# WangYuTum/odometry

Measured on AMD Instinct MI355X. Metric: tracked frames/sec (1241x376, 4-level pyramid), higher is better.
Workload: dtype f32

## Files before the change

### __graft_entry__.py

```python
import os
import sys

ROOT = os.path.dirname(os.path.abspath(__file__))
if ROOT not in sys.path:
    sys.path.insert(0, ROOT)


def build():
    import subprocess
    from odometry_amd import build as b
    b.build(force=False, verbose=True)
    from oracle import oracle
    oracle.build()
    subprocess.check_call(["g++", "-O2", "-std=c++17", "-ffp-contract=off", "-fno-fast-math", "-mfma", "-shared", "-fPIC",
                           "-o", os.path.join(ROOT, "tests", "_build_hostemu.so"), os.path.join(ROOT, "tests", "hostemu.cpp")])
    import importlib.util
    spec = importlib.util.spec_from_file_location("devmath", os.path.join(ROOT, "tests", "devmath.py"))
    devmath = importlib.util.module_from_spec(spec)
    spec.loader.exec_module(devmath)
    devmath.build_all(verbose=True)
    import odometry_amd
    from odometry_amd import _lib
    _lib.load()


def smoke():
    import numpy as np
    from odometry_amd import api, synth
    from oracle import oracle as O
    seq = synth.make_sequence(2, seed=5, with_depth=True)
    L0, L1, R1 = seq["left"][0], seq["left"][1], seq["right"][1]
    inv = synth.semi_dense_inverse_depth(seq["depth"][0], L0)
    p0, d0, p1 = api.ImagePyramid(4, L0, True), api.DepthPyramid(4, inv, False), api.ImagePyramid(4, L1, True)
    for l, ref in enumerate(O.image_pyramid(L1, 4, True)):
        assert np.array_equal(p1.GetPyramidImage(l), ref), f"pyramid level {l} differs from the oracle"
    lm = api.LevenbergMarquardtOptimizer(0.01, 0.995, [10, 20, 30, 30], np.eye(4), None, 1, 28.0)
    T = lm.Solve(p0, d0, p1)
    ref = O.lm_solve(O.image_pyramid(L0, flat=True), O.depth_pyramid(inv, flat=True), O.image_pyramid(L1, flat=True),
                     376, 1241, O.lm_params())
    assert lm.last_status == 0 and ref["status"] == 0
    err = float(np.abs(T.astype(np.float64) - ref["pose"]).max())
    assert err < 1e-5, f"pose differs from the oracle by {err}"
    de = api.DepthEstimator(8.0, 900.0, 15.0, 0.1, 30.0, 0.01, 28.0, 0.995, 50, 4, None, None,
                            float(np.float32(386.1448) / np.float32(718.856)), 80000)
    val = np.zeros(L1.shape, np.uint8)
    disp = np.zeros(L1.shape, np.float32)
    dep = np.zeros(L1.shape, np.float32)
    st = de.ComputeDepth(L1, R1, val, disp, dep)
    rd = O.compute_depth(L1, R1, O.depth_params())
    assert st == rd["status"] == 0
    assert np.array_equal(disp, rd["disp"]) and np.array_equal(val, rd["val"])
    print(f"smoke ok: pose max|d|={err:.2e}, evals={lm.launch_stats()[0]}, valid depth={int(val.sum())}")


if __name__ == "__main__":
    build()
    if len(sys.argv) > 1 and sys.argv[1] == "smoke":
        smoke()
```

### odometry_amd/csrc/kernels.hip.h

```cpp
#pragma once
#include <hip/hip_runtime.h>
#include "odo_math.h"

#ifndef ODO_PHASE_STAMPS
#define ODO_PHASE_STAMPS 0
#endif
#if ODO_PHASE_STAMPS
#define ODO_DBG(a) ((a).dbg)
#else
#define ODO_DBG(a) ((unsigned long long*)nullptr)
#endif

#ifndef ODO_KERNEL
#define ODO_KERNEL __global__
#define ODO_KERNEL_T __global__
#endif
#ifdef ODO_LM_CHAIN_TU
#define ODO_DEVICE_VAR static __device__
#else
#define ODO_DEVICE_VAR __device__
#endif

namespace odo {

// ... 987 lines not shown
    if (pending) need_step = lm_decide(&s, acc_sh, precision);
    if (smdbg) { c1 = __builtin_readcyclecounter(); c2 = c1; c3 = c1; }
    if (need_step) {
      float d[6];
      solve_damped_wave_regs(acc_sh, s.lambda, d);
#pragma unroll
      for (int i = 0; i < 6; i++) s.delta[i] = d[i];
      if (smdbg) { asm volatile("" ::"v"(d[0]), "v"(d[5])); c2 = __builtin_readcyclecounter(); }
#ifdef ODO_NO_LANE_SINCOS
      lm_apply_step(&s, s.max_iters);
#else
      lm_apply_step_wave(&s, s.max_iters);
#endif
      if (smdbg) { asm volatile("" ::"v"(s.T[0]), "v"(s.T[14])); c3 = __builtin_readcyclecounter(); }
    }
    if (smdbg && t == 0) { smdbg[0] += c1 - c0; smdbg[1] += c2 - c1; smdbg[2] += c3 - c2; smdbg[3] += 1; }
    if (pending) {
      if (publisher && t == 0 && trace) {
        const int ev = s.n_evals - 1;
        if (ev < kTraceCap) {
          LmTraceRow& r = trace[ev];
          r.level = lvl0;
          r.iter = iter0;
          r.n_res = (int)acc_sh[28];
          r.err = s.err_now;
          r.accepted = (s.status == 0 && !(s.err_now > err_last0)) ? 1 : 0;
          r.stop = (s.stop_reason == 3 || s.active) ? 0 : s.stop_reason;
          r.lambda_after = s.lambda;
#pragma unroll
          for (int i = 0; i < 6; i++) r.delta[i] = (s.active || s.stop_reason == 3) ? s.delta[i] : 0.0f;
        }
        int evals_this_level = 0;
#pragma unroll
        for (int i = 0; i < 8; i++) evals_this_level += (i == (lvl0 & 7)) ? s.iters_level[i] : 0;
        if (iter0 == 0 && evals_this_level == 1) cost_stat[lvl0 * 2 + 0] = s.err_now;
        cost_stat[lvl0 * 2 + 1] = s.err_now;
      }
      s.pending = 0;
    }
    if (lv) {
      while (!s.active && s.status == 0 && !s.finished) {
        const int next = (s.level < 0) ? n_levels - 1 : s.level - 1;
        if (next < stop_level) { s.finished = 1; break; }
        s.stop_reason = 0;
        lm_begin_level(&s, next, lambda0, lv[next].max_iters);
      }
      if (s.status != 0) s.finished = 1;
    }
    if (t == 0) s_sh = s;
  }
  __syncthreads();
}

struct LmHot {
  Se3 cur, inc;
  float Tc[12];
  float lambda, err_last;
  int level, iter, max_iters, active, status, finished, n_evals, stop_reason;
};
__device__ __forceinline__ void lm_hot_load(LmHot& h, const LmState& s) {
  h.cur = s.cur; h.inc = s.inc;
  float M[16];
  se3_to_colmajor(s.cur, M);
#pragma unroll
  for (int c = 0; c < 4; c++)
#pragma unroll
    for (int r = 0; r < 3; r++) h.Tc[c * 3 + r] = M[c * 4 + r];
  h.lambda = s.lambda; h.err_last = s.err_last;
  h.level = s.level; h.iter = s.iter; h.max_iters = s.max_iters; h.active = s.active; h.status = s.status; h.finished = s.finished;
  h.n_evals = s.n_evals; h.stop_reason = s.stop_reason;
}
__device__ __forceinline__ void lm_hot_store(const LmHot& h, LmState& s) {
  s.cur = h.cur; s.inc = h.inc; s.last = h.cur;
  s.lambda = h.lambda; s.err_last = h.err_last;
  s.level = h.level; s.iter = h.iter; s.max_iters = h.max_iters; s.active = h.active; s.status = h.status; s.finished = h.finished;
  s.n_evals = h.n_evals; s.stop_reason = h.stop_reason;
  s.pending = 0;
}
__device__ __forceinline__ void lm_state_machine_hot(LmHot& h, const StepLevel* lv, int n_levels, float lambda0, float precision,
                                                     LmState& s_sh, const double* acc_sh, LmTraceRow* __restrict__ trace,
                                                     float* __restrict__ cost_stat, bool publisher,
                                                     unsigned long long* smdbg = nullptr, int stop_level = 0) {
  const int t = threadIdx.x;
  if (t < 64) {
    unsigned long long c0 = smdbg ? __builtin_readcyclecounter() : 0, c1 = c0, c2 = c0, c3 = c0;
    const int iter0 = h.iter, lvl0 = h.level;
    const float err_last0 = h.err_last;
    float Tprev[12];
#pragma unroll
    for (int c = 0; c < 4; c++)
#pragma unroll
      for (int r = 0; r < 3; r++) Tprev[c * 3 + r] = s_sh.T[c * 4 + r];
    h.n_evals++;
    if (t == 0) s_sh.iters_level[lvl0 & 7] += 1;
    bool need_step = false;
    float err_now = 0.0f;
    bool have_err = false;
    if (!(acc_sh[28] > 0.0)) {
      h.status = -1;
      h.active = 0;
    } else {
      err_now = (float)(acc_sh[27] / acc_sh[28]);
      have_err = true;
      if (err_now > h.err_last) {
        h.lambda = h.lambda * 5.0f;
        if (h.lambda > 1e+5f) { h.active = 0; h.stop_reason = 2; }
        else need_step = true;
      } else {
        h.cur = h.inc;
#pragma unroll
        for (int i = 0; i < 12; i++) h.Tc[i] = Tprev[i];
        const float err_diff = err_now / h.err_last;
        if (err_diff > precision) { h.active = 0; h.stop_reason = 1; }
        else {
          h.err_last = err_now;
          h.lambda = fmaxf(h.lambda / 5.0f, 1e-5f);
          need_step = true;
        }
      }
    }
    if (smdbg) { c1 = __builtin_readcyclecounter(); c2 = c1; c3 = c1; }
    float d[6] = {0.0f, 0.0f, 0.0f, 0.0f, 0.0f, 0.0f};
    bool new_T = false;
    float Tn[16];
#pragma unroll
    for (int i = 0; i < 16; i++) Tn[i] = 0.0f;
    if (need_step) {
      solve_damped_wave_regs(acc_sh, h.lambda, d);
      if (smdbg) { asm volatile("" ::"v"(d[0]), "v"(d[5])); c2 = __builtin_readcyclecounter(); }
      Se3 dd;
      se3_exp_wave(d, &dd);
      const float C[16] = {h.Tc[0], h.Tc[1], h.Tc[2], 0.0f, h.Tc[3], h.Tc[4], h.Tc[5], 0.0f,
                           h.Tc[6], h.Tc[7], h.Tc[8], 0.0f, h.Tc[9], h.Tc[10], h.Tc[11], 1.0f};
      se3_left_update_mat(dd, C, &h.inc);
      se3_to_colmajor(h.inc, Tn);
      new_T = true;
      h.iter++;
      if (!(h.max_iters > h.iter)) { h.active = 0; h.stop_reason = 3; }
      if (smdbg) { asm volatile("" ::"v"(Tn[0]), "v"(Tn[14])); c3 = __builtin_readcyclecounter(); }
    }
    if (smdbg && t == 0) { smdbg[0] += c1 - c0; smdbg[1] += c2 - c1; smdbg[2] += c3 - c2; smdbg[3] += 1; }
    if (t == 0) {
      if (have_err) s_sh.err_now = err_now;
      if (need_step) {
#pragma unroll
        for (int i = 0; i < 6; i++) s_sh.delta[i] = d[i];
      }
    }
    if (publisher && t == 0 && trace) {
      const int ev = h.n_evals - 1;
      const float e = s_sh.err_now;
      if (ev < kTraceCap) {
        LmTraceRow& r = trace[ev];
        r.level = lvl0;
        r.iter = iter0;
        r.n_res = (int)acc_sh[28];
        r.err = e;
        r.accepted = (h.status == 0 && !(e > err_last0)) ? 1 : 0;
        r.stop = (h.stop_reason == 3 || h.active) ? 0 : h.stop_reason;
        r.lambda_after = h.lambda;
#pragma unroll
        for (int i = 0; i < 6; i++) r.delta[i] = (h.active || h.stop_reason == 3) ? d[i] : 0.0f;
      }
      const int evals_this_level = s_sh.iters_level[lvl0 & 7];
      if (iter0 == 0 && evals_this_level == 1) cost_stat[lvl0 * 2 + 0] = e;
      cost_stat[lvl0 * 2 + 1] = e;
    }
    if (lv) {
      while (!h.active && h.status == 0 && !h.finished) {
        const int next = (h.level < 0) ? n_levels - 1 : h.level - 1;
        if (next < stop_level) { h.finished = 1; break; }
        h.stop_reason = 0;
        h.level = next;
        h.iter = 0;
        h.err_last = 1e+10f;
        h.lambda = lambda0;
        h.inc = h.cur;
        h.max_iters = lv[next].max_iters;
        h.active = (h.status == 0 && h.max_iters > 0) ? 1 : 0;
#pragma unroll
        for (int c = 0; c < 4; c++) {
#pragma unroll
          for (int r = 0; r < 3; r++) Tn[c * 4 + r] = h.Tc[c * 3 + r];
          Tn[c * 4 + 3] = (c == 3) ? 1.0f : 0.0f;
        }
        new_T = true;
      }
      if (h.status != 0) h.finished = 1;
    }
    if (t == 0) {
      if (new_T) {
#pragma unroll
        for (int i = 0; i < 16; i++) s_sh.T[i] = Tn[i];
      }
      s_sh.level = h.level; s_sh.active = h.active; s_sh.status = h.status; s_sh.finished = h.finished;
    }
  }
  __syncthreads();
}

constexpr int kUpdThreads = 1024;
#define ODO_STAMP(i) do { if (STAMP && threadIdx.x == 0) stamps[i] = __builtin_readcyclecounter(); } while (0)
template <bool STAMP>
__device__ __forceinline__ void lm_update_body(LmState* __restrict__ st, const double* __restrict__ partials,
                                               int nblk, int expect_level, float precision, int max_iters,
                                               LmTraceRow* __restrict__ trace, float* __restrict__ cost_stat,
                                               int* __restrict__ host_prog, int seq,
                                               unsigned long long* __restrict__ stamps) {
  ODO_STAMP(0);
  if (!(st->active != 0 && st->level == expect_level)) {
    if (host_prog && threadIdx.x == 0) __hip_atomic_store(host_prog, seq, __ATOMIC_RELAXED, __HIP_MEMORY_SCOPE_SYSTEM);
    return;
  }
  __shared__ double sh[32][32];
  __shared__ double acc_sh[32];
  __shared__ LmState s_sh;
  const int t = threadIdx.x;
  const int q = t & 31, seg = t >> 5;
  double v = 0.0;
  if (q < ODO_NACC) {
    double v0 = 0.0, v1 = 0.0, v2 = 0.0, v3 = 0.0;
    int b = seg;
    for (; b + 96 < nblk; b += 128) {
      v0 += partials[(size_t)b * ODO_NACC + q];
      v1 += partials[(size_t)(b + 32) * ODO_NACC + q];
      v2 += partials[(size_t)(b + 64) * ODO_NACC + q];
      v3 += partials[(size_t)(b + 96) * ODO_NACC + q];
    }
    for (; b < nblk; b += 32) v0 += partials[(size_t)b * ODO_NACC + q];
    v = (v0 + v1) + (v2 + v3);
  }
  ODO_STAMP(1);
  sh[seg][q] = v;
  if (t < (int)(sizeof(LmState) / sizeof(int))) ((int*)&s_sh)[t] = ((const int*)st)[t];
  __syncthreads();
  if (t < ODO_NACC) {
    double a = 0.0;
#pragma unroll
    for (int g = 0; g < 32; g++) a += sh[g][t];
    acc_sh[t] = a;
  }
  if (t == 0) s_sh.max_iters = max_iters;
  __syncthreads();
  ODO_STAMP(2);
  lm_state_machine(true, nullptr, 0, 0.0f, precision, s_sh, acc_sh, trace, cost_stat, true);
  ODO_STAMP(3); ODO_STAMP(4); ODO_STAMP(5); ODO_STAMP(6);
  if (t < (int)(sizeof(LmState) / sizeof(int))) ((int*)st)[t] = ((const int*)&s_sh)[t];
  if (t == 0) {
    const LmState& s = s_sh;
    if (host_prog) {
      if (!s.active) __hip_atomic_store(host_prog + 2 + expect_level, 1, __ATOMIC_RELAXED, __HIP_MEMORY_SCOPE_SYSTEM);
// ... 254 lines not shown
  lm_span_begin(q.span);
  __shared__ LmState s_sh;
  extern __shared__ __attribute__((aligned(16))) double red_sh[];
  __shared__ double acc_sh[32];
  __shared__ StepLevel lv_sh[ODO_MAX_LEVELS_K];
  __shared__ unsigned long long sm_sh[4];
  unsigned long long arm_g0 = 0;
  if (kArmed && threadIdx.x < 17) arm_g0 = __hip_atomic_load(a.arm + threadIdx.x, __ATOMIC_RELAXED, __HIP_MEMORY_SCOPE_SYSTEM);
  lm_copy_levels(lv_sh, lv_src);
  if (threadIdx.x == 0) {
#pragma unroll
    for (int i = 0; i < 4; i++) sm_sh[i] = 0;
  }
  __shared__ __attribute__((aligned(16))) float arm_pose_sh[16];
  __shared__ __attribute__((aligned(16))) int arm_verdict_sh4[4];
  if (kArmed) {
    if (threadIdx.x < 64) {
      const int lane = (int)threadIdx.x;
      unsigned long long g = arm_g0;
      bool got = __all(lane >= 17 || (int)(g >> 32) == a.token);
      const unsigned long long t0 = (unsigned long long)wall_clock64();
      for (int spin = 0; !got; spin++) {
        if (lane < 17) g = __hip_atomic_load(a.arm + lane, __ATOMIC_RELAXED, __HIP_MEMORY_SCOPE_SYSTEM);
        got = __all(lane >= 17 || (int)(g >> 32) == a.token);
        if (!got && (spin & 15) == 15 && (unsigned long long)wall_clock64() - t0 > (a.fine_wait ? (unsigned long long)a.fine_wait : kArmWaitTicks)) break;
      }
      if (lane < 16) arm_pose_sh[lane] = __uint_as_float((unsigned)g);
      if (lane == 16) arm_verdict_sh4[0] = got ? (int)(unsigned)g : 3;
    }
    __syncthreads();
    if (arm_verdict_sh4[0] == 3) {
      if (threadIdx.x < 64) {
        if (threadIdx.x < (int)(sizeof(LmState) / sizeof(int))) ((int*)&s_sh)[threadIdx.x] = 0;
        if (threadIdx.x == 0) { s_sh.status = -2; s_sh.active = 0; s_sh.finished = 1; }
      }
      __syncthreads();
      lm_fused_publish(s_sh, q.st_out, a.host_prog, q.seq, a.token, a.cost_stat, a.out, a.done_flag, a.final_state);
      return;
    }
    if (arm_verdict_sh4[0] != 1) return;
  } else {
    __syncthreads();
  }
#if ODO_PHASE_STAMPS
  const unsigned long long w_p1 = (unsigned long long)wall_clock64();
#endif
  lm_fused_prologue(q.st_in, q.part_in, lv_sh, a.n_levels, a.lambda0, a.precision, s_sh, red_sh, acc_sh, (kFull ? a.trace : (LmTraceRow*)nullptr), a.cost_stat, true,
                    kArmed ? arm_pose_sh : (q.first_of_solve ? a.init : nullptr), a.stop_level, (!kArmed && a.chain_in_token) ? a.chain_pose : nullptr);
#if ODO_PHASE_STAMPS
  const unsigned long long w_p2 = (unsigned long long)wall_clock64();
#endif
  LmHot hot;
  lm_hot_load(hot, s_sh);
  if (ODO_DBG(a) && threadIdx.x == 0 && q.seq < 56) ODO_DBG(a)[16 + 2 * q.seq] = wall_clock64();
  unsigned long long c_eval = 0, c_red = 0, c_sm = 0, c_it = 0, c_last = ODO_DBG(a) ? __builtin_readcyclecounter() : 0;
  const unsigned long long c_begin = c_last, w_begin = ODO_DBG(a) ? (unsigned long long)wall_clock64() : 0;
  auto lap = [&](unsigned long long& sum) {
    if (ODO_DBG(a)) { const unsigned long long now = __builtin_readcyclecounter(); sum += now - c_last; c_last = now; }
  };
  static_assert(kCoarseBlock == 2 * kLmBlock, "two 256-point virtual blocks per round");
  constexpr int kS = 8;
  constexpr int kVbMax = (kCoarseMaxPoints + kLmBlock - 1) / kLmBlock;
  __shared__ double part_sh[kVbMax][32];
  __shared__ double sc_part[2][kCoarseChunks];
  __shared__ int sc_cnt[kCoarseChunks];
  const int tl = threadIdx.x & (kLmBlock - 1), half = threadIdx.x >> 8;
  float* rows_sh = (float*)red_sh + half * (kRowFloats * RowBuf<kLmBlock>::W);
  const int my_q = tl / kS, my_s = tl % kS;
  int rowA = 0, rowB = 0;
  if (my_q < ODO_NACC) rows_of_quantity(my_q, &rowA, &rowB);
  PointK cpt[kCoarseRounds];
  bool cpt_ok[kCoarseRounds] = {false, false};
  int cpt_level = -1;
  for (int guard = 0; guard < 4096; guard++) {
    const bool run = (s_sh.active != 0 && s_sh.status == 0 && s_sh.level >= min_level);
    if (!run) break;
    c_it++;
    const StepLevel& L = lv_sh[s_sh.level];
    const float* I2u = lm_uniform_ptr(L.I2);
    float T[16];
#pragma unroll
    for (int i = 0; i < 16; i++) T[i] = s_sh.T[i];
    const int nvb = L.nblk;
    if (s_sh.level != cpt_level) {
      cpt_level = s_sh.level;
#pragma unroll
      for (int rd = 0; rd < kCoarseRounds; rd++) {
        const int vb = 2 * rd + half, idx = vb * kLmBlock + tl;
        cpt_ok[rd] = vb < nvb && idx < L.n;
        if (cpt_ok[rd]) cpt[rd] = load_point(L.pl, idx);
      }
    }
    float td_r[kCoarseRounds] = {0.0f, 0.0f}, td_J[kCoarseRounds][6] = {{0.0f, 0.0f, 0.0f, 0.0f, 0.0f, 0.0f}, {0.0f, 0.0f, 0.0f, 0.0f, 0.0f, 0.0f}};
    bool td_valid[kCoarseRounds] = {false, false};
    float td_scale_sqr = 1.0f;
    if ((kFull && a.robust == 2)) {
      float e2[kCoarseRounds];
#pragma unroll
      for (int rd = 0; rd < kCoarseRounds; rd++) {
        if (cpt_ok[rd]) td_valid[rd] = point_residual_g<kFull>(cpt[rd], T, L.k, I2u, L.rows, L.cols, &td_r[rd], td_J[rd]);
        e2[rd] = td_r[rd] * td_r[rd];
      }
      const float sg = coarse_tdist_sigma(sc_part, sc_cnt, e2, td_valid, (nvb + 1) / 2);
      td_scale_sqr = sg * sg;
    }
#pragma unroll
    for (int vb0 = 0; vb0 < 2 * kCoarseRounds; vb0 += 2) {
      if (vb0 >= nvb) break;
      const int vb = vb0 + half;
      float r = 0.0f, w = 0.0f, J[6] = {0.0f, 0.0f, 0.0f, 0.0f, 0.0f, 0.0f};
      bool valid = false;
      if ((kFull && a.robust == 2)) {
        r = td_r[vb0 / 2]; valid = td_valid[vb0 / 2];
#pragma unroll
        for (int i = 0; i < 6; i++) J[i] = td_J[vb0 / 2][i];
        if (valid) w = robust_weight(r, 2, a.huber_delta, td_scale_sqr);
      } else if (cpt_ok[vb0 / 2]) {
        if (point_residual_g<kFull>(cpt[vb0 / 2], T, L.k, I2u, L.rows, L.cols, &r, J)) {
          w = robust_weight(r, kFull ? a.robust : (a.robust == 1 ? 1 : 0), a.huber_delta, 1.0f);
          valid = true;
        }
      }
      if (vb0 > 0) __syncthreads();
      rows_store_z(rows_sh, RowBuf<kLmBlock>::W, tl, J, w, r, valid);
      __syncthreads();
      if (vb0 == 0) lap(c_eval);
      double accq = 0.0;
      if (vb < nvb) {
        if (my_q < ODO_NACC) accq = rows_accumulate<kLmBlock, kS>(rows_sh, rowA, rowB, my_s, accq);
        accq = rows_butterfly8(accq);
      }
      if (nvb == 1) {
        if (half == 0 && my_q < ODO_NACC && my_s == 0) {
          double v = 0.0;
          v += accq;
          double acc = 0.0;
          acc += v;
#pragma unroll
          for (int g = 1; g < 8; g++) acc += 0.0;
          acc_sh[my_q] = acc;
        }
      } else if (vb < nvb && my_q < ODO_NACC && my_s == 0) {
        part_sh[vb][my_q] = accq;
      }
    }
    __syncthreads();
    if (nvb > 1) {
      const int fq = threadIdx.x & 31, fseg = threadIdx.x >> 5;
      double* fold_sh = red_sh;
      if (fseg < 8) {
        double v = 0.0;
        if (fq < ODO_NACC)
          for (int b = fseg; b < nvb; b += 8) v += part_sh[b][fq];
        fold_sh[fseg * 32 + fq] = v;
      }
      __syncthreads();
      if (threadIdx.x < ODO_NACC) {
        double acc = 0.0;
#pragma unroll
        for (int g = 0; g < 8; g++) acc += fold_sh[g * 32 + threadIdx.x];
        acc_sh[threadIdx.x] = acc;
      }
    }
    lap(c_red);
    lm_state_machine_hot(hot, lv_sh, a.n_levels, a.lambda0, a.precision, s_sh, acc_sh, (kFull ? a.trace : (LmTraceRow*)nullptr), a.cost_stat, true,
                         ODO_DBG(a) ? sm_sh : nullptr, a.stop_level);
    lap(c_sm);
  }
#if ODO_PHASE_STAMPS
  const unsigned long long w_loop_end = (unsigned long long)wall_clock64();
#endif
  if (threadIdx.x == 0) lm_hot_store(hot, s_sh);
  lm_fused_publish(s_sh, q.st_out, a.host_prog, q.seq, a.token, a.cost_stat, a.out, a.done_flag, a.final_state, chain_out_of(a));
#if ODO_PHASE_STAMPS
  if (ODO_DBG(a) && threadIdx.x == 0) {
    const unsigned long long now = (unsigned long long)wall_clock64();
    g_lm_diag[4] += w_begin - w_entry; g_lm_diag[5] += w_loop_end - w_begin; g_lm_diag[6] += now - w_loop_end;
    g_lm_diag[16] += w_p1 - w_entry; g_lm_diag[17] += w_p2 - w_p1; g_lm_diag[18] += w_begin - w_p2;
    if (g_lm_diag[1] && w_entry > g_lm_diag[1] && w_entry - g_lm_diag[1] < 100000ull) { g_lm_diag[7] += w_entry - g_lm_diag[1]; g_lm_diag[3] += w_entry - g_lm_diag[2]; g_lm_diag[14] += 1; }
    g_lm_diag[0] = now; g_lm_diag[8] += 1;
  }
#endif
  if (ODO_DBG(a) && threadIdx.x == 0) {
    if (q.seq < 56) ODO_DBG(a)[16 + 2 * q.seq + 1] = wall_clock64();
    ODO_DBG(a)[0] += c_eval; ODO_DBG(a)[1] += c_red; ODO_DBG(a)[2] += c_sm; ODO_DBG(a)[3] += c_it;
    ODO_DBG(a)[4] += __builtin_readcyclecounter() - c_begin; ODO_DBG(a)[5] += 1;
    ODO_DBG(a)[6] += (unsigned long long)wall_clock64() - w_begin;
#pragma unroll
    for (int i = 0; i < 4; i++) ODO_DBG(a)[8 + i] += sm_sh[i];
  }
  lm_span_end(q.span);
}

#ifdef ODO_LM_CHAIN_TU
static __global__ void __launch_bounds__(kCoarseBlock) lm_coarse_kernel(StepArgs a, int min_level) {
  const StepLaunch q = {a.st_in, a.st_out, a.part_in, a.part_out, a.seq, a.first_of_solve, a.span};
  lm_coarse_body<false>(a, q, min_level, lm_kernarg_words());
}
static __global__ void __launch_bounds__(kCoarseBlock) lm_coarse_armed_kernel(StepArgs a, int min_level) {
  const StepLaunch q = {a.st_in, a.st_out, a.part_in, a.part_out, a.seq, a.first_of_solve, a.span};
  lm_coarse_body<false, true>(a, q, min_level, lm_kernarg_words());
}
static __global__ void __launch_bounds__(kCoarseBlock) lm_coarse_full_kernel(StepArgs a, int min_level) {
  const StepLaunch q = {a.st_in, a.st_out, a.part_in, a.part_out, a.seq, a.first_of_solve, a.span};
  lm_coarse_body<true>(a, q, min_level, lm_kernarg_words());
}
#endif
template <bool kFull>
__device__ __forceinline__ void lm_coarse_batch_entry(const StepArgs* __restrict__ table, int seq, int first_of_solve, unsigned long long* span) {
  const StepArgs& a = table[blockIdx.y];
  const StepLaunch q = {a.st2[seq & 1], a.st2[(seq + 1) & 1], a.part2[seq & 1], a.part2[(seq + 1) & 1], seq, first_of_solve, span};
  lm_coarse_body<kFull>(a, q, a.min_level, (const unsigned*)&table[blockIdx.y]);
}
ODO_KERNEL void __launch_bounds__(kCoarseBlock) lm_coarse_kernel_batch(const StepArgs* __restrict__ table, int seq, int first_of_solve,
                                                                       unsigned long long* span) {
  lm_coarse_batch_entry<false>(table, seq, first_of_solve, span);
}
ODO_KERNEL void __launch_bounds__(kCoarseBlock) lm_coarse_full_kernel_batch(const StepArgs* __restrict__ table, int seq, int first_of_solve,
                                                                            unsigned long long* span) {
  lm_coarse_batch_entry<true>(table, seq, first_of_solve, span);
}

constexpr int kFineGran = 2 * ODO_NACC;
constexpr int kFineRowsMax = 160;
constexpr int kFineChunk = 8;
// ... 197 lines not shown
  return sigma;
}
template <bool kTdist, bool kTrace>
__device__ __forceinline__ void lm_fine_body(const StepArgs& a, const StepLaunch& q, int K, int w, unsigned long long* __restrict__ xbuf,
                                             int fault, int lo_level, const unsigned* __restrict__ lv_src) {
#if ODO_PHASE_STAMPS
  const unsigned long long w_entry = (unsigned long long)wall_clock64();
#endif
  __builtin_amdgcn_s_setprio(3);
  const int t = threadIdx.x, tl = t & (kLmBlock - 1), half = t >> 8;
  const bool publisher = (w == 0);
  if (publisher && t == 0 && q.span) atomicMin(q.span, (unsigned long long)wall_clock64());
  __shared__ LmState s_sh;
  __shared__ double fold_sh[8 * 32];
  __shared__ double acc_sh[32];
  __shared__ StepLevel lv_sh[ODO_MAX_LEVELS_K];
  __shared__ float rows_sh2[2][kRowFloats * RowBuf<kLmBlock>::W];
  __shared__ int bail_sh, local_sh;
  __shared__ unsigned long long sm_sh[4];
  float* rows_sh = rows_sh2[half];
  const unsigned tag_base = a.fine_epoch << 8;
  unsigned long long* place = xbuf + 2 * kFineRowsMax * kFineGran;
  const unsigned wait_limit = a.fine_wait ? a.fine_wait : kFineWaitTicks;
  lm_copy_levels(lv_sh, lv_src);
  if (t == 0) {
    bail_sh = 0;
    local_sh = 0;
#pragma unroll
    for (int i = 0; i < 4; i++) sm_sh[i] = 0;
    __hip_atomic_store(place + w, ((unsigned long long)(unsigned)fine_xcc_id() << 32) | tag_base, __ATOMIC_RELAXED, __HIP_MEMORY_SCOPE_AGENT);
  }
  __syncthreads();
  lm_fused_prologue(q.st_in, q.part_in, lv_sh, a.n_levels, a.lambda0, a.precision, s_sh, fold_sh, acc_sh, (kTrace ? a.trace : (LmTraceRow*)nullptr), a.cost_stat,
                    publisher, q.first_of_solve ? a.init : nullptr, a.stop_level, a.chain_in_token ? a.chain_pose : nullptr);
  LmHot hot;
  lm_hot_load(hot, s_sh);
  if (t < 64) {
    bool same = true, got = false;
    if (t < K) {
      unsigned long long pw = 0;
      const FineDeadline dl = FineDeadline::begin(wait_limit);
      for (int spin = 0; !got; spin++) {
        pw = __hip_atomic_load(place + t, __ATOMIC_RELAXED, __HIP_MEMORY_SCOPE_AGENT);
        got = ((unsigned)pw == tag_base);
        if (!got && dl.expired(spin)) break;
      }
      same = got && ((int)(pw >> 32) == fine_xcc_id());
    } else {
      got = true;
    }
    const bool all_got = __all(got), all_same = __all(same);
    if (t == 0) { local_sh = (all_got && all_same) ? 1 : 0; if (!all_got) bail_sh = 1; }
  }
  __syncthreads();
  const bool local = local_sh != 0;
  constexpr int kS = 8;
  const int my_q = tl / kS, my_s = tl % kS;
  int rowA = 0, rowB = 0;
  if (my_q < ODO_NACC) rows_of_quantity(my_q, &rowA, &rowB);
  const int fq = t & 31, fseg = t >> 5;
  PointK pt;
  bool pt_ok = false;
  int pt_level = -1;
  unsigned long long c_eval = 0, c_xchg = 0, c_sm = 0, c_it = 0, c_last = ODO_DBG(a) ? __builtin_readcyclecounter() : 0;
#if ODO_PHASE_STAMPS
  unsigned long long c_first = 0, n_first = 0;
#endif
  const unsigned long long c_begin = c_last, w_begin = ODO_DBG(a) ? (unsigned long long)wall_clock64() : 0;
  auto lap = [&](unsigned long long& sum) {
    if (ODO_DBG(a)) { const unsigned long long now = __builtin_readcyclecounter(); sum += now - c_last; c_last = now; }
  };
  for (int ev = 0; ev < 4096; ev++) {
    const bool run = (s_sh.active != 0 && s_sh.status == 0 && !s_sh.finished && !bail_sh && s_sh.level >= lo_level);
    if (!run) break;
    c_it++;
    const StepLevel& L = lv_sh[s_sh.level];
    const float* I2u = lm_uniform_ptr(L.I2);
    const int nblk = L.nblk;
    const unsigned tag = tag_base + 1u + (unsigned)(ev % 255);
    unsigned long long* buf = xbuf + (size_t)(ev & 1) * kFineRowsMax * kFineGran;
    float T[16];
#pragma unroll
    for (int i = 0; i < 16; i++) T[i] = s_sh.T[i];
#if ODO_PHASE_STAMPS
    const bool first_of_level = (s_sh.level != pt_level);
#endif
    const bool resident = (nblk <= 2 * K) && (L.n <= nblk * kLmBlock);
    if (resident) {
      const int vb = w + half * K;
      if (s_sh.level != pt_level) {
        pt_level = s_sh.level;
        const int idx = vb * kLmBlock + tl;
        pt_ok = vb < nblk && idx < L.n;
        if (pt_ok) pt = load_point(L.pl, idx);
      }
      float r = 0.0f, wgt = 0.0f, J[6] = {0.0f, 0.0f, 0.0f, 0.0f, 0.0f, 0.0f};
      bool valid = false;
      if (pt_ok && point_residual_g<kTdist || kTrace>(pt, T, L.k, I2u, L.rows, L.cols, &r, J)) {
        wgt = robust_weight(r, (kTdist || kTrace) ? a.robust : (a.robust == 1 ? 1 : 0), a.huber_delta, 1.0f);
        valid = true;
      }
      if (kTdist && w < nblk) {
        __shared__ double td_ws_sh[2][8];
        __shared__ int td_cnt_sh[8];
        const float sg = fine_tdist_sigma(xbuf + kFineScaleOff, vb * 4 + (tl >> 6), 4 * nblk,
                                          ((a.fine_epoch & 0xfffu) << 20) | (((unsigned)ev & 0x3ffu) << 10), r * r, valid, local, wait_limit, &bail_sh,
                                          td_ws_sh, td_cnt_sh);
        if (valid) wgt = robust_weight(r, 2, a.huber_delta, sg * sg);
      }
      rows_store_z(rows_sh, RowBuf<kLmBlock>::W, tl, J, wgt, r, valid);
      __syncthreads();
      if (bail_sh) break;
      if (vb < nblk) {
        double accq = 0.0;
        if (my_q < ODO_NACC) accq = rows_accumulate<kLmBlock, kS>(rows_sh, rowA, rowB, my_s, accq);
        accq = rows_butterfly8(accq);
        if (my_q < ODO_NACC && my_s == 0 && !(fault && vb == 0)) fine_publish(buf, vb, my_q, accq, tag, local);
      }
    } else {
      const int rounds = (L.n + nblk * kLmBlock - 1) / (nblk * kLmBlock);
      for (int vb0 = w; vb0 < nblk; vb0 += 2 * K) {
        const int vb = vb0 + half * K;
        double accq = 0.0;
        for (int rd = 0; rd < rounds; rd++) {
          const int idx = (vb + rd * nblk) * kLmBlock + tl;
          float r = 0.0f, wgt = 0.0f, J[6] = {0.0f, 0.0f, 0.0f, 0.0f, 0.0f, 0.0f};
          bool valid = false;
          if (vb < nblk && idx < L.n) {
            const PointK p = load_point(L.pl, idx);
            if (point_residual_g<kTdist || kTrace>(p, T, L.k, I2u, L.rows, L.cols, &r, J)) {
              wgt = robust_weight(r, (kTdist || kTrace) ? a.robust : (a.robust == 1 ? 1 : 0), a.huber_delta, 1.0f);
              valid = true;
            }
          }
          __syncthreads();
          rows_store_z(rows_sh, RowBuf<kLmBlock>::W, tl, J, wgt, r, valid);
          __syncthreads();
          if (my_q < ODO_NACC) accq = rows_accumulate<kLmBlock, kS>(rows_sh, rowA, rowB, my_s, accq);
        }
        accq = rows_butterfly8(accq);
        if (vb < nblk && my_q < ODO_NACC && my_s == 0 && !(fault && vb == 0)) fine_publish(buf, vb, my_q, accq, tag, local);
      }
    }
#if ODO_PHASE_STAMPS
    { const unsigned long long before = c_eval; lap(c_eval); if (first_of_level) { c_first += c_eval - before; n_first++; } }
#else
    lap(c_eval);
#endif
    double v = 0.0;
    __builtin_amdgcn_s_setprio(0);
    if (fq < ODO_NACC && fseg < 8) {
      for (int b0 = fseg; b0 < nblk; b0 += 8 * kFineChunk) {
        FineG2 g2[kFineChunk];
        bool all = false;
        FineDeadline dl = {0ull, 0ull, wait_limit};
        for (int spin = 0; !all; spin++) {
          if (spin == 1) dl = FineDeadline::begin(wait_limit);
          if (spin > 0) { if (dl.expired(spin)) break; __builtin_amdgcn_s_sleep(1); }
          all = true;
#pragma unroll
          for (int u = 0; u < kFineChunk; u++) {
            const int b = b0 + 8 * u;
            if (b < nblk) g2[u] = *(const volatile FineG2Global*)(buf + (size_t)b * kFineGran + 2 * fq);
          }
#pragma unroll
          for (int u = 0; u < kFineChunk; u++) {
            const int b = b0 + 8 * u;
            if (b < nblk) all = all && (g2[u].x == tag) && (g2[u].z == tag);
          }
        }
        if (!all) bail_sh = 1;
#pragma unroll
        for (int u = 0; u < kFineChunk; u++) {
          const int b = b0 + 8 * u;
          if (b < nblk) v += __longlong_as_double((long long)(((unsigned long long)g2[u].y << 32) | (unsigned long long)g2[u].w));
        }
      }
    }
    __builtin_amdgcn_s_setprio(3);
    if (fseg < 8) fold_sh[fseg * 32 + fq] = v;
    __syncthreads();
    if (t < ODO_NACC) {
      double acc = 0.0;
#pragma unroll
      for (int g = 0; g < 8; g++) acc += fold_sh[g * 32 + t];
      acc_sh[t] = acc;
    }
    lap(c_xchg);
    if (bail_sh) break;
    lm_state_machine_hot(hot, lv_sh, a.n_levels, a.lambda0, a.precision, s_sh, acc_sh, (kTrace ? a.trace : (LmTraceRow*)nullptr), a.cost_stat, publisher,
                         (ODO_DBG(a) && publisher) ? sm_sh : nullptr, a.stop_level);
    lap(c_sm);
  }
#if ODO_PHASE_STAMPS
  const unsigned long long w_loop_end = (unsigned long long)wall_clock64();
#endif
  if (t == 0) lm_hot_store(hot, s_sh);
  if (bail_sh && t == 0) { s_sh.status = -2; s_sh.active = 0; s_sh.finished = 1; }
  __syncthreads();
  if (publisher) {
    lm_fused_publish(s_sh, q.st_out, a.host_prog, q.seq, a.token, a.cost_stat, a.out, a.done_flag, a.final_state, chain_out_of(a));
#if ODO_PHASE_STAMPS
    const unsigned long long w_published = (unsigned long long)wall_clock64();
#endif
    if (ODO_DBG(a) && t == 0) { ODO_DBG(a)[128] += c_eval; ODO_DBG(a)[129] += c_xchg; ODO_DBG(a)[130] += c_sm; ODO_DBG(a)[131] += c_it; ODO_DBG(a)[132] += 1; ODO_DBG(a)[133] += local ? 1 : 0;
      ODO_DBG(a)[134] += __builtin_readcyclecounter() - c_begin; ODO_DBG(a)[135] += (unsigned long long)wall_clock64() - w_begin;
#pragma unroll
      for (int i = 0; i < 4; i++) ODO_DBG(a)[136 + i] += sm_sh[i]; }
    if (t == 0 && q.span) atomicMax(q.span + 1, (unsigned long long)wall_clock64());
#if ODO_PHASE_STAMPS
    if (ODO_DBG(a) && t == 0) {
      const unsigned long long now = w_published;
      g_lm_diag[2] = w_loop_end;
      g_lm_diag[19] += c_first; g_lm_diag[20] += n_first;
      g_lm_diag[9] += w_begin - w_entry; g_lm_diag[10] += w_loop_end - w_begin; g_lm_diag[11] += now - w_loop_end;
      if (g_lm_diag[0] && w_entry > g_lm_diag[0] && w_entry - g_lm_diag[0] < 100000ull) { g_lm_diag[12] += w_entry - g_lm_diag[0]; g_lm_diag[15] += 1; }
      g_lm_diag[1] = now; g_lm_diag[13] += 1;
    }
#endif
  }
}
ODO_DEVICE_VAR unsigned g_lm_fine_dispatch[2];
__device__ __forceinline__ bool lm_fine_mid_dispatch() {
  return __hip_atomic_load(&g_lm_fine_dispatch[0], __ATOMIC_RELAXED, __HIP_MEMORY_SCOPE_AGENT) !=
         __hip_atomic_load(&g_lm_fine_dispatch[1], __ATOMIC_RELAXED, __HIP_MEMORY_SCOPE_AGENT);
}
template <bool kTdist, bool kTrace>
__device__ __forceinline__ void lm_fine_entry(const StepArgs& a, int K, unsigned long long* __restrict__ xbuf, int fault, int lo_level,
                                              unsigned* dispatch_words) {
  if (threadIdx.x == 0) {
    if (blockIdx.x == 0) __hip_atomic_store(&dispatch_words[0], a.fine_dispatch, __ATOMIC_RELAXED, __HIP_MEMORY_SCOPE_AGENT);
    if (blockIdx.x == gridDim.x - 1) __hip_atomic_store(&dispatch_words[1], a.fine_dispatch, __ATOMIC_RELAXED, __HIP_MEMORY_SCOPE_AGENT);
  }
  if (!fine_on_home(a.fine_home) || lm_chain_skip(a)) return;
  const StepLaunch q = {a.st_in, a.st_out, a.part_in, a.part_out, a.seq, a.first_of_solve, a.span};
  lm_fine_body<kTdist, kTrace>(a, q, K, (int)(blockIdx.x >> 3), xbuf, fault, lo_level, lm_kernarg_words());
}
#ifdef ODO_LM_CHAIN_TU
static __global__ void __launch_bounds__(kFineThreads) lm_fine_kernel(StepArgs a, int K, unsigned long long* __restrict__ xbuf, int fault,
                                                               int lo_level, unsigned* dispatch_words) {
  lm_fine_entry<false, false>(a, K, xbuf, fault, lo_level, dispatch_words);
}
static __global__ void __launch_bounds__(kFineThreads) lm_fine_trace_kernel(StepArgs a, int K, unsigned long long* __restrict__ xbuf, int fault,
                                                                     int lo_level, unsigned* dispatch_words) {
  lm_fine_entry<false, true>(a, K, xbuf, fault, lo_level, dispatch_words);
}
static __global__ void __launch_bounds__(kFineThreads) lm_fine_tdist_kernel(StepArgs a, int K, unsigned long long* __restrict__ xbuf, int fault,
                                                                     int lo_level, unsigned* dispatch_words) {
  lm_fine_entry<true, true>(a, K, xbuf, fault, lo_level, dispatch_words);
}
// ... 846 lines not shown
```

Measured before the change: 4063.

## Pack LM loop state into compact shared packet and carry handover state in registers

Introduces a compact shared LmPacket holding the 3x4 pose, the current level constants and a packed control word, so each LM loop iteration reads one small struct instead of scattered LmState fields and the level table. Per-level eval counts, err_now and delta are carried in registers instead of being written to shared memory each iteration. Lambda up/down candidates are precomputed during the reduction wait, and the fine-exchange spin delays arming its deadline. The aim is a shorter serial state-machine and loop-head path between evaluations, at the cost of more register pressure and more complex state write-back.

```diff
diff --git a/__graft_entry__.py b/__graft_entry__.py
--- a/__graft_entry__.py
+++ b/__graft_entry__.py
@@ -19,6 +19,18 @@
     devmath = importlib.util.module_from_spec(spec)
     spec.loader.exec_module(devmath)
     devmath.build_all(verbose=True)
+    tests_dir = os.path.join(ROOT, "tests")
+    sys.path.insert(0, tests_dir)
+    try:
+        spec = importlib.util.spec_from_file_location("handover", os.path.join(tests_dir, "handover.py"))
+        handover = importlib.util.module_from_spec(spec)
+        spec.loader.exec_module(handover)
+        procs = [(subprocess.Popen(handover.command(u)), u) for u in handover.UNITS if handover.stale(u)]
+        for pr, u in procs:
+            if pr.wait() != 0:
+                raise subprocess.CalledProcessError(pr.returncode, handover.command(u))
+    finally:
+        sys.path.remove(tests_dir)
     import odometry_amd
     from odometry_amd import _lib
     _lib.load()
diff --git a/odometry_amd/csrc/kernels.hip.h b/odometry_amd/csrc/kernels.hip.h
--- a/odometry_amd/csrc/kernels.hip.h
+++ b/odometry_amd/csrc/kernels.hip.h
@@ -1063,11 +1063,79 @@
   __syncthreads();
 }
 
+#ifndef ODO_HO_DELTA_REGS
+#define ODO_HO_DELTA_REGS 0
+#endif
+#ifndef ODO_HO_CHAIN
+#define ODO_HO_CHAIN 15
+#endif
+#ifndef ODO_HO_MAIN
+#define ODO_HO_MAIN 15
+#endif
+#ifdef ODO_LM_CHAIN_TU
+constexpr int kHoMask = ODO_HO_CHAIN;
+#else
+constexpr int kHoMask = ODO_HO_MAIN;
+#endif
+constexpr bool kHoEarly = (kHoMask & 1) != 0, kHoRetry = (kHoMask & 2) != 0, kHoPacket = (kHoMask & 4) != 0, kHoCarry = (kHoMask & 8) != 0;
+struct __attribute__((aligned(16))) LmPacket {
+  float T[12];
+  StepLevel L;
+  int ctl;
+  int pad_[1];
+};
+static_assert(sizeof(StepLevel) % 4 == 0 && offsetof(LmPacket, L) % 8 == 0, "LmPacket: StepLevel copied by dwords");
+__device__ __forceinline__ int lm_packet_ctl(int level, int active, int status, int finished) {
+  return (level & 0xff) | (active != 0 ? 0x100 : 0) | (status == 0 ? 0x200 : 0) | (finished != 0 ? 0x400 : 0);
+}
+__device__ __forceinline__ int lm_packet_level(int ctl) { return (int)(signed char)(ctl & 0xff); }
+__device__ __forceinline__ bool lm_packet_run(int ctl, bool unfinished) {
+  return (ctl & (unfinished ? 0x700 : 0x300)) == 0x300;
+}
+__device__ __forceinline__ void lm_packet_fill(LmPacket& pk, const LmState& s_sh, const StepLevel* lv_sh) {
+  const int t = threadIdx.x;
+  constexpr int kLevelWords = (int)(sizeof(StepLevel) / sizeof(unsigned));
+  const int lvl = s_sh.level;
+  if (t < 12) pk.T[t] = s_sh.T[(t / 3) * 4 + (t % 3)];
+  if (t == 12) pk.ctl = lm_packet_ctl(lvl, s_sh.active, s_sh.status, s_sh.finished);
+  if (t >= 16 && t < 16 + kLevelWords && lvl >= 0) ((unsigned*)&pk.L)[t - 16] = ((const unsigned*)&lv_sh[lvl])[t - 16];
+}
+struct LmLevelConsts { int n, nblk, rows, cols; LevelK k; const float* I2; };
+struct LmLoopHead { float T[16]; int ctl, level; LmLevelConsts c; };
+__device__ __forceinline__ void lm_loop_head(LmLoopHead& H, const LmPacket& pk) {
+#pragma unroll
+  for (int c = 0; c < 4; c++) {
+#pragma unroll
+    for (int r = 0; r < 3; r++) H.T[c * 4 + r] = pk.T[c * 3 + r];
+    H.T[c * 4 + 3] = (c == 3) ? 1.0f : 0.0f;
+  }
+  H.c.n = pk.L.n; H.c.nblk = pk.L.nblk; H.c.rows = pk.L.rows; H.c.cols = pk.L.cols; H.c.k = pk.L.k;
+  unsigned long long i2 = (unsigned long long)pk.L.I2;
+  H.ctl = pk.ctl;
+  asm volatile("" : "+v"(H.T[0]), "+v"(H.T[14]), "+v"(H.c.n), "+v"(H.c.nblk), "+v"(H.c.rows), "+v"(H.c.cols), "+v"(H.c.k.fl), "+v"(H.c.k.cx),
+               "+v"(H.c.k.cy), "+v"(i2), "+v"(H.ctl));
+  H.c.I2 = (const float*)i2;
+  H.level = lm_packet_level(H.ctl);
+}
+__device__ __forceinline__ void lm_loop_head(LmLoopHead& H, const LmState& s_sh, const StepLevel* lv_sh) {
+  H.level = s_sh.level;
+  H.ctl = lm_packet_ctl(H.level, s_sh.active, s_sh.status, s_sh.finished);
+#pragma unroll
+  for (int i = 0; i < 16; i++) H.T[i] = s_sh.T[i];
+  const StepLevel& L = lv_sh[H.level & (ODO_MAX_LEVELS_K - 1)];
+  H.c.n = L.n; H.c.nblk = L.nblk; H.c.rows = L.rows; H.c.cols = L.cols; H.c.k = L.k; H.c.I2 = L.I2;
+}
 struct LmHot {
   Se3 cur, inc;
   float Tc[12];
   float lambda, err_last;
   int level, iter, max_iters, active, status, finished, n_evals, stop_reason;
+  float err_now;
+#if ODO_HO_DELTA_REGS
+  float delta[6];
+#endif
+  int evals_level;
+  float lam_up, lam_dn;
 };
 __device__ __forceinline__ void lm_hot_load(LmHot& h, const LmState& s) {
   h.cur = s.cur; h.inc = s.inc;
@@ -1080,19 +1148,41 @@
   h.lambda = s.lambda; h.err_last = s.err_last;
   h.level = s.level; h.iter = s.iter; h.max_iters = s.max_iters; h.active = s.active; h.status = s.status; h.finished = s.finished;
   h.n_evals = s.n_evals; h.stop_reason = s.stop_reason;
+  h.err_now = s.err_now;
+#if ODO_HO_DELTA_REGS
+#pragma unroll
+  for (int i = 0; i < 6; i++) h.delta[i] = s.delta[i];
+#endif
+  h.evals_level = kHoCarry ? s.iters_level[s.level & 7] : 0;
+  h.lam_up = 0.0f; h.lam_dn = 0.0f;
 }
 __device__ __forceinline__ void lm_hot_store(const LmHot& h, LmState& s) {
   s.cur = h.cur; s.inc = h.inc; s.last = h.cur;
   s.lambda = h.lambda; s.err_last = h.err_last;
   s.level = h.level; s.iter = h.iter; s.max_iters = h.max_iters; s.active = h.active; s.status = h.status; s.finished = h.finished;
   s.n_evals = h.n_evals; s.stop_reason = h.stop_reason;
+  if (kHoCarry) {
+    s.err_now = h.err_now;
+#if ODO_HO_DELTA_REGS
+#pragma unroll
+    for (int i = 0; i < 6; i++) s.delta[i] = h.delta[i];
+#endif
+    s.iters_level[h.level & 7] = h.evals_level;
+  }
   s.pending = 0;
 }
-__device__ __forceinline__ void lm_state_machine_hot(LmHot& h, const StepLevel* lv, int n_levels, float lambda0, float precision,
+__device__ __forceinline__ void lm_hot_candidates(LmHot& h) {
+  h.lam_up = h.lambda * 5.0f;
+  h.lam_dn = fmaxf(h.lambda / 5.0f, 1e-5f);
+  asm volatile("" : "+v"(h.lam_up), "+v"(h.lam_dn));
+}
+template <bool kEarly = false>
+__device__ __forceinline__ bool lm_state_machine_hot(LmHot& h, const StepLevel* lv, int n_levels, float lambda0, float precision,
                                                      LmState& s_sh, const double* acc_sh, LmTraceRow* __restrict__ trace,
                                                      float* __restrict__ cost_stat, bool publisher,
-                                                     unsigned long long* smdbg = nullptr, int stop_level = 0) {
+                                                     unsigned long long* smdbg = nullptr, int stop_level = 0, LmPacket* pk = nullptr) {
   const int t = threadIdx.x;
+  bool wrote_T = false;
   if (t < 64) {
     unsigned long long c0 = smdbg ? __builtin_readcyclecounter() : 0, c1 = c0, c2 = c0, c3 = c0;
     const int iter0 = h.iter, lvl0 = h.level;
@@ -1101,9 +1191,11 @@
 #pragma unroll
     for (int c = 0; c < 4; c++)
 #pragma unroll
-      for (int r = 0; r < 3; r++) Tprev[c * 3 + r] = s_sh.T[c * 4 + r];
+      for (int r = 0; r < 3; r++) Tprev[c * 3 + r] = pk ? pk->T[c * 3 + r] : s_sh.T[c * 4 + r];
     h.n_evals++;
-    if (t == 0) s_sh.iters_level[lvl0 & 7] += 1;
+    if (kHoCarry) h.evals_level++;
+    else if (t == 0) s_sh.iters_level[lvl0 & 7] += 1;
+    const float lam_up = kEarly ? h.lam_up : h.lambda * 5.0f;
     bool need_step = false;
     float err_now = 0.0f;
     bool have_err = false;
@@ -1114,7 +1206,7 @@
       err_now = (float)(acc_sh[27] / acc_sh[28]);
       have_err = true;
       if (err_now > h.err_last) {
-        h.lambda = h.lambda * 5.0f;
+        h.lambda = lam_up;
         if (h.lambda > 1e+5f) { h.active = 0; h.stop_reason = 2; }
         else need_step = true;
       } else {
@@ -1125,11 +1217,12 @@
         if (err_diff > precision) { h.active = 0; h.stop_reason = 1; }
         else {
           h.err_last = err_now;
-          h.lambda = fmaxf(h.lambda / 5.0f, 1e-5f);
+          h.lambda = kEarly ? h.lam_dn : fmaxf(h.lambda / 5.0f, 1e-5f);
           need_step = true;
         }
       }
     }
+    if (kHoCarry && have_err) h.err_now = err_now;
     if (smdbg) { c1 = __builtin_readcyclecounter(); c2 = c1; c3 = c1; }
     float d[6] = {0.0f, 0.0f, 0.0f, 0.0f, 0.0f, 0.0f};
     bool new_T = false;
@@ -1138,6 +1231,15 @@
     for (int i = 0; i < 16; i++) Tn[i] = 0.0f;
     if (need_step) {
       solve_damped_wave_regs(acc_sh, h.lambda, d);
+#if ODO_HO_DELTA_REGS
+#pragma unroll
+      for (int i = 0; i < 6; i++) h.delta[i] = d[i];
+#else
+      if (kHoCarry && t == 0) {
+#pragma unroll
+        for (int i = 0; i < 6; i++) s_sh.delta[i] = d[i];
+      }
+#endif
       if (smdbg) { asm volatile("" ::"v"(d[0]), "v"(d[5])); c2 = __builtin_readcyclecounter(); }
       Se3 dd;
       se3_exp_wave(d, &dd);
@@ -1151,7 +1253,7 @@
       if (smdbg) { asm volatile("" ::"v"(Tn[0]), "v"(Tn[14])); c3 = __builtin_readcyclecounter(); }
     }
     if (smdbg && t == 0) { smdbg[0] += c1 - c0; smdbg[1] += c2 - c1; smdbg[2] += c3 - c2; smdbg[3] += 1; }
-    if (t == 0) {
+    if (!kHoCarry && t == 0) {
       if (have_err) s_sh.err_now = err_now;
       if (need_step) {
 #pragma unroll
@@ -1160,7 +1262,7 @@
     }
     if (publisher && t == 0 && trace) {
       const int ev = h.n_evals - 1;
-      const float e = s_sh.err_now;
+      const float e = kHoCarry ? h.err_now : s_sh.err_now;
       if (ev < kTraceCap) {
         LmTraceRow& r = trace[ev];
         r.level = lvl0;
@@ -1173,7 +1275,7 @@
 #pragma unroll
         for (int i = 0; i < 6; i++) r.delta[i] = (h.active || h.stop_reason == 3) ? d[i] : 0.0f;
       }
-      const int evals_this_level = s_sh.iters_level[lvl0 & 7];
+      const int evals_this_level = kHoCarry ? h.evals_level : s_sh.iters_level[lvl0 & 7];
       if (iter0 == 0 && evals_this_level == 1) cost_stat[lvl0 * 2 + 0] = e;
       cost_stat[lvl0 * 2 + 1] = e;
     }
@@ -1198,16 +1300,45 @@
         new_T = true;
       }
       if (h.status != 0) h.finished = 1;
-    }
-    if (t == 0) {
+      if (kHoCarry && h.level != lvl0) {
+        if (t == 0) s_sh.iters_level[lvl0 & 7] = h.evals_level;
+        h.evals_level = s_sh.iters_level[h.level & 7];
+      }
+    }
+    if (pk) {
+      if (h.level != lvl0 && h.level >= 0) {
+        constexpr int kLevelWords = (int)(sizeof(StepLevel) / sizeof(unsigned));
+        if (t < kLevelWords) ((unsigned*)&pk->L)[t] = ((const unsigned*)&lv[h.level])[t];
+      }
+      if (t == 0) {
+        if (new_T) {
+#pragma unroll
+          for (int c = 0; c < 4; c++)
+#pragma unroll
+            for (int r = 0; r < 3; r++) pk->T[c * 3 + r] = Tn[c * 4 + r];
+        }
+        pk->ctl = lm_packet_ctl(h.level, h.active, h.status, h.finished);
+      }
+    } else if (t == 0) {
       if (new_T) {
 #pragma unroll
         for (int i = 0; i < 16; i++) s_sh.T[i] = Tn[i];
       }
       s_sh.level = h.level; s_sh.active = h.active; s_sh.status = h.status; s_sh.finished = h.finished;
     }
+    wrote_T = new_T && t == 0;
   }
   __syncthreads();
+  return wrote_T;
+}
+__device__ __forceinline__ void lm_packet_T_out(const LmPacket& pk, LmState& s_sh, bool wrote_T) {
+  if (!wrote_T) return;
+#pragma unroll
+  for (int c = 0; c < 4; c++) {
+#pragma unroll
+    for (int r = 0; r < 3; r++) s_sh.T[c * 4 + r] = pk.T[c * 3 + r];
+    s_sh.T[c * 4 + 3] = (c == 3) ? 1.0f : 0.0f;
+  }
 }
 
 constexpr int kUpdThreads = 1024;
@@ -1568,6 +1699,12 @@
 #endif
   LmHot hot;
   lm_hot_load(hot, s_sh);
+  __shared__ LmPacket pk_sh;
+  bool wrote_T = false;
+  if (kHoPacket) {
+    lm_packet_fill(pk_sh, s_sh, lv_sh);
+    __syncthreads();
+  }
   if (ODO_DBG(a) && threadIdx.x == 0 && q.seq < 56) ODO_DBG(a)[16 + 2 * q.seq] = wall_clock64();
   unsigned long long c_eval = 0, c_red = 0, c_sm = 0, c_it = 0, c_last = ODO_DBG(a) ? __builtin_readcyclecounter() : 0;
   const unsigned long long c_begin = c_last, w_begin = ODO_DBG(a) ? (unsigned long long)wall_clock64() : 0;
@@ -1589,17 +1726,19 @@
   bool cpt_ok[kCoarseRounds] = {false, false};
   int cpt_level = -1;
   for (int guard = 0; guard < 4096; guard++) {
-    const bool run = (s_sh.active != 0 && s_sh.status == 0 && s_sh.level >= min_level);
+    LmLoopHead H;
+    if (kHoPacket) lm_loop_head(H, pk_sh);
+    else lm_loop_head(H, s_sh, lv_sh);
+    const bool run = (lm_packet_run(H.ctl, false) && H.level >= min_level);
     if (!run) break;
     c_it++;
-    const StepLevel& L = lv_sh[s_sh.level];
-    const float* I2u = lm_uniform_ptr(L.I2);
-    float T[16];
-#pragma unroll
-    for (int i = 0; i < 16; i++) T[i] = s_sh.T[i];
-    const int nvb = L.nblk;
-    if (s_sh.level != cpt_level) {
-      cpt_level = s_sh.level;
+    const StepLevel& L = kHoPacket ? pk_sh.L : lv_sh[H.level];
+    const LmLevelConsts& Lc = H.c;
+    const float* I2u = lm_uniform_ptr(Lc.I2);
+    const float* T = H.T;
+    const int nvb = Lc.nblk;
+    if (H.level != cpt_level) {
+      cpt_level = H.level;
 #pragma unroll
       for (int rd = 0; rd < kCoarseRounds; rd++) {
         const int vb = 2 * rd + half, idx = vb * kLmBlock + tl;
@@ -1614,7 +1753,7 @@
       float e2[kCoarseRounds];
 #pragma unroll
       for (int rd = 0; rd < kCoarseRounds; rd++) {
-        if (cpt_ok[rd]) td_valid[rd] = point_residual_g<kFull>(cpt[rd], T, L.k, I2u, L.rows, L.cols, &td_r[rd], td_J[rd]);
+        if (cpt_ok[rd]) td_valid[rd] = point_residual_g<kFull>(cpt[rd], T, Lc.k, I2u, Lc.rows, Lc.cols, &td_r[rd], td_J[rd]);
         e2[rd] = td_r[rd] * td_r[rd];
       }
       const float sg = coarse_tdist_sigma(sc_part, sc_cnt, e2, td_valid, (nvb + 1) / 2);
@@ -1632,13 +1771,14 @@
         for (int i = 0; i < 6; i++) J[i] = td_J[vb0 / 2][i];
         if (valid) w = robust_weight(r, 2, a.huber_delta, td_scale_sqr);
       } else if (cpt_ok[vb0 / 2]) {
-        if (point_residual_g<kFull>(cpt[vb0 / 2], T, L.k, I2u, L.rows, L.cols, &r, J)) {
+        if (point_residual_g<kFull>(cpt[vb0 / 2], T, Lc.k, I2u, Lc.rows, Lc.cols, &r, J)) {
           w = robust_weight(r, kFull ? a.robust : (a.robust == 1 ? 1 : 0), a.huber_delta, 1.0f);
           valid = true;
         }
       }
       if (vb0 > 0) __syncthreads();
       rows_store_z(rows_sh, RowBuf<kLmBlock>::W, tl, J, w, r, valid);
+      if (kHoEarly && vb0 == 0) lm_hot_candidates(hot);
       __syncthreads();
       if (vb0 == 0) lap(c_eval);
       double accq = 0.0;
@@ -1679,14 +1819,17 @@
       }
     }
     lap(c_red);
-    lm_state_machine_hot(hot, lv_sh, a.n_levels, a.lambda0, a.precision, s_sh, acc_sh, (kFull ? a.trace : (LmTraceRow*)nullptr), a.cost_stat, true,
-                         ODO_DBG(a) ? sm_sh : nullptr, a.stop_level);
+    wrote_T |= lm_state_machine_hot<kHoEarly>(hot, lv_sh, a.n_levels, a.lambda0, a.precision, s_sh, acc_sh, (kFull ? a.trace : (LmTraceRow*)nullptr), a.cost_stat, true,
+                                              ODO_DBG(a) ? sm_sh : nullptr, a.stop_level, kHoPacket ? &pk_sh : nullptr);
     lap(c_sm);
   }
 #if ODO_PHASE_STAMPS
   const unsigned long long w_loop_end = (unsigned long long)wall_clock64();
 #endif
-  if (threadIdx.x == 0) lm_hot_store(hot, s_sh);
+  if (threadIdx.x == 0) {
+    lm_hot_store(hot, s_sh);
+    if (kHoPacket) lm_packet_T_out(pk_sh, s_sh, wrote_T);
+  }
   lm_fused_publish(s_sh, q.st_out, a.host_prog, q.seq, a.token, a.cost_stat, a.out, a.done_flag, a.final_state, chain_out_of(a));
 #if ODO_PHASE_STAMPS
   if (ODO_DBG(a) && threadIdx.x == 0) {
@@ -1990,8 +2133,12 @@
     const bool all_got = __all(got), all_same = __all(same);
     if (t == 0) { local_sh = (all_got && all_same) ? 1 : 0; if (!all_got) bail_sh = 1; }
   }
+  __shared__ LmPacket pk_sh;
+  bool wrote_T = false;
+  if (kHoPacket) lm_packet_fill(pk_sh, s_sh, lv_sh);
   __syncthreads();
   const bool local = local_sh != 0;
+  const bool bail0 = bail_sh != 0;
   constexpr int kS = 8;
   const int my_q = tl / kS, my_s = tl % kS;
   int rowA = 0, rowB = 0;
@@ -2009,32 +2156,34 @@
     if (ODO_DBG(a)) { const unsigned long long now = __builtin_readcyclecounter(); sum += now - c_last; c_last = now; }
   };
   for (int ev = 0; ev < 4096; ev++) {
-    const bool run = (s_sh.active != 0 && s_sh.status == 0 && !s_sh.finished && !bail_sh && s_sh.level >= lo_level);
+    LmLoopHead H;
+    if (kHoPacket) lm_loop_head(H, pk_sh);
+    else lm_loop_head(H, s_sh, lv_sh);
+    const bool run = (lm_packet_run(H.ctl, true) && !bail0 && H.level >= lo_level);
     if (!run) break;
     c_it++;
-    const StepLevel& L = lv_sh[s_sh.level];
-    const float* I2u = lm_uniform_ptr(L.I2);
-    const int nblk = L.nblk;
+    const StepLevel& L = kHoPacket ? pk_sh.L : lv_sh[H.level];
+    const LmLevelConsts& Lc = H.c;
+    const float* I2u = lm_uniform_ptr(Lc.I2);
+    const int nblk = Lc.nblk;
     const unsigned tag = tag_base + 1u + (unsigned)(ev % 255);
     unsigned long long* buf = xbuf + (size_t)(ev & 1) * kFineRowsMax * kFineGran;
-    float T[16];
-#pragma unroll
-    for (int i = 0; i < 16; i++) T[i] = s_sh.T[i];
+    const float* T = H.T;
 #if ODO_PHASE_STAMPS
-    const bool first_of_level = (s_sh.level != pt_level);
-#endif
-    const bool resident = (nblk <= 2 * K) && (L.n <= nblk * kLmBlock);
+    const bool first_of_level = (H.level != pt_level);
+#endif
+    const bool resident = (nblk <= 2 * K) && (Lc.n <= nblk * kLmBlock);
     if (resident) {
       const int vb = w + half * K;
-      if (s_sh.level != pt_level) {
-        pt_level = s_sh.level;
+      if (H.level != pt_level) {
+        pt_level = H.level;
         const int idx = vb * kLmBlock + tl;
-        pt_ok = vb < nblk && idx < L.n;
+        pt_ok = vb < nblk && idx < Lc.n;
         if (pt_ok) pt = load_point(L.pl, idx);
       }
       float r = 0.0f, wgt = 0.0f, J[6] = {0.0f, 0.0f, 0.0f, 0.0f, 0.0f, 0.0f};
       bool valid = false;
-      if (pt_ok && point_residual_g<kTdist || kTrace>(pt, T, L.k, I2u, L.rows, L.cols, &r, J)) {
+      if (pt_ok && point_residual_g<kTdist || kTrace>(pt, T, Lc.k, I2u, Lc.rows, Lc.cols, &r, J)) {
         wgt = robust_weight(r, (kTdist || kTrace) ? a.robust : (a.robust == 1 ? 1 : 0), a.huber_delta, 1.0f);
         valid = true;
       }
@@ -2056,7 +2205,7 @@
         if (my_q < ODO_NACC && my_s == 0 && !(fault && vb == 0)) fine_publish(buf, vb, my_q, accq, tag, local);
       }
     } else {
-      const int rounds = (L.n + nblk * kLmBlock - 1) / (nblk * kLmBlock);
+      const int rounds = (Lc.n + nblk * kLmBlock - 1) / (nblk * kLmBlock);
       for (int vb0 = w; vb0 < nblk; vb0 += 2 * K) {
         const int vb = vb0 + half * K;
         double accq = 0.0;
@@ -2064,9 +2213,9 @@
           const int idx = (vb + rd * nblk) * kLmBlock + tl;
           float r = 0.0f, wgt = 0.0f, J[6] = {0.0f, 0.0f, 0.0f, 0.0f, 0.0f, 0.0f};
           bool valid = false;
-          if (vb < nblk && idx < L.n) {
+          if (vb < nblk && idx < Lc.n) {
             const PointK p = load_point(L.pl, idx);
-            if (point_residual_g<kTdist || kTrace>(p, T, L.k, I2u, L.rows, L.cols, &r, J)) {
+            if (point_residual_g<kTdist || kTrace>(p, T, Lc.k, I2u, Lc.rows, Lc.cols, &r, J)) {
               wgt = robust_weight(r, (kTdist || kTrace) ? a.robust : (a.robust == 1 ? 1 : 0), a.huber_delta, 1.0f);
               valid = true;
             }
@@ -2086,6 +2235,7 @@
     lap(c_eval);
 #endif
     double v = 0.0;
+    if (kHoEarly) lm_hot_candidates(hot);
     __builtin_amdgcn_s_setprio(0);
     if (fq < ODO_NACC && fseg < 8) {
       for (int b0 = fseg; b0 < nblk; b0 += 8 * kFineChunk) {
@@ -2093,7 +2243,7 @@
         bool all = false;
         FineDeadline dl = {0ull, 0ull, wait_limit};
         for (int spin = 0; !all; spin++) {
-          if (spin == 1) dl = FineDeadline::begin(wait_limit);
+          if (spin == (kHoRetry ? 8 : 1)) dl = FineDeadline::begin(wait_limit);
           if (spin > 0) { if (dl.expired(spin)) break; __builtin_amdgcn_s_sleep(1); }
           all = true;
 #pragma unroll
@@ -2126,14 +2276,17 @@
     }
     lap(c_xchg);
     if (bail_sh) break;
-    lm_state_machine_hot(hot, lv_sh, a.n_levels, a.lambda0, a.precision, s_sh, acc_sh, (kTrace ? a.trace : (LmTraceRow*)nullptr), a.cost_stat, publisher,
-                         (ODO_DBG(a) && publisher) ? sm_sh : nullptr, a.stop_level);
+    wrote_T |= lm_state_machine_hot<kHoEarly>(hot, lv_sh, a.n_levels, a.lambda0, a.precision, s_sh, acc_sh, (kTrace ? a.trace : (LmTraceRow*)nullptr), a.cost_stat, publisher,
+                                              (ODO_DBG(a) && publisher) ? sm_sh : nullptr, a.stop_level, kHoPacket ? &pk_sh : nullptr);
     lap(c_sm);
   }
 #if ODO_PHASE_STAMPS
   const unsigned long long w_loop_end = (unsigned long long)wall_clock64();
 #endif
-  if (t == 0) lm_hot_store(hot, s_sh);
+  if (t == 0) {
+    lm_hot_store(hot, s_sh);
+    if (kHoPacket) lm_packet_T_out(pk_sh, s_sh, wrote_T);
+  }
   if (bail_sh && t == 0) { s_sh.status = -2; s_sh.active = 0; s_sh.finished = 1; }
   __syncthreads();
   if (publisher) {
```

After: 4015. 1.2% lower.
